# cvlab-kaist/CoPoNeRF

Measured on AMD Instinct MI355X. Metric: rendered rays/sec (RealEstate10K-shaped 256x256 stereo pair, full-image render, 64 samples/ray), higher is better.
Workload: dtype f16 (fp16-input/fp32-accumulate MFMA for the per-sample MLPs; f32 decoder; f64 geometry island); 1 GPU; configs[1]: 256x256 stereo pair (narrow rig), full-image render 65536 rays x 64 samples, 1 pair(s) per GPU, render path only (z/rel_pose/flow given, val=True); chunk_rays=65536, lanes=1, pairs_per_gpu=1

## Files before the change

### coponerf_amd/csrc/attend_units.hip

```cpp
#include <algorithm>

#include "hid_sum.h"
#include "local_units_body.h"

namespace {

constexpr int HC = 1664;
constexpr int NCHUNK = HC / 8;
constexpr int NL = 4;
constexpr int NS = 2 * TG;
constexpr int AU_THREADS = (NL + NS) * 64;
constexpr int RU = HID_BLOCK_ROWS;
constexpr int LDS_MAX = 160 * 1024;

__device__ __forceinline__ float wave_max(float v) {
#pragma unroll
    for (int o = 32; o > 0; o >>= 1) v = fmaxf(v, __shfl_xor(v, o));
    return v;
}
__device__ __forceinline__ float wave_sum(float v) {
#pragma unroll
    for (int o = 32; o > 0; o >>= 1) v += __shfl_xor(v, o);
    return v;
}
__device__ __forceinline__ void group_barrier() {
    asm volatile("s_waitcnt lgkmcnt(0)" ::: "memory");
    __builtin_amdgcn_s_barrier();
    asm volatile("" ::: "memory");
}

struct GroupUnits {
    unsigned lw, upg, upw, nmy, bid, nwg;
    __device__ __forceinline__ unsigned niter() const { return nmy * upw; }
    __device__ __forceinline__ unsigned unit(unsigned it, int, bool& live) const {
        it = min(it, nmy * upw - 1);
        const unsigned k = it / upw, idx = lw + (it - k * upw) * NL;
        live = idx < upg;
        return (bid + k * nwg) * upg + min(idx, upg - 1);
    }
    __device__ __forceinline__ void after(unsigned it) const {
        if ((it + 1) % upw == 0) group_barrier();
    }
};
struct RingLogits {
    float* ring;
    float* __restrict__ logits;
    unsigned lw, upw, nsblk;
    int S, T, a, fg;
    __device__ __forceinline__ void operator()(unsigned it, int, long long srow, float d) const {
        if (srow < 0 || fg != 0) return;
        const unsigned k = it / upw, idx = lw + (it - k * upw) * NL;
        const int v = (int)(idx / nsblk), s = (int)(idx % nsblk) * TSW + (a >> 2);
        ring[(k & 1) * (TG * T) + (a & 3) * T + v * S + s] = d;
        if (logits) logits[srow] = d;
    }
};

template <int MODE>
__global__ __launch_bounds__(AU_THREADS, 3) void attend_units_kernel(UnitArgs args, UnitGeo geo, const __half* __restrict__ hid,
                                                                     __half* __restrict__ hbar, float* __restrict__ at_wt,
                                                                     float* __restrict__ logits) {
    extern __shared__ __attribute__((aligned(16))) char smem[];
    constexpr size_t WB = 8 * 4 * 64 * sizeof(half8);
    UnitLds L;
    L.w2l = reinterpret_cast<half8*>(smem);
    L.wkl = reinterpret_cast<half8*>(smem + WB);
    L.b2s = reinterpret_cast<float*>(smem + 2 * WB);
    L.bks = L.b2s + 128;
    L.w1s = reinterpret_cast<half4*>(L.bks + 128);
    const int V = geo.V, R = geo.R, S = geo.S, T = V * S;
    float* ring = reinterpret_cast<float*>(smem + unit_lds_bytes<MODE>());
    float* wbuf = ring + 2 * TG * T;
    const int lane = threadIdx.x & 63;
    const int wave = __builtin_amdgcn_readfirstlane((int)(threadIdx.x >> 6));

    unit_stage_weights<MODE>(L, args, (int)threadIdx.x, AU_THREADS);
    __syncthreads();

    const unsigned upg = (unsigned)(V * geo.nsblk);
    const unsigned ngroups = (unsigned)geo.nunits / upg;
    const unsigned bid = blockIdx.x, nwg = gridDim.x;
    const unsigned nmy = (ngroups - bid + nwg - 1) / nwg;

    if (wave < NL) {
        const unsigned upw = (upg + NL - 1) / NL;
        GroupUnits seq{(unsigned)wave, upg, upw, nmy, bid, nwg};
        RingLogits sink{ring, logits, (unsigned)wave, upw, (unsigned)geo.nsblk, S, T, lane & 15, lane >> 4};
        unit_walk<MODE, 1>(L, args, geo, lane, seq, sink);
        return;
    }

    __builtin_amdgcn_s_setprio(1);
    const int sw = wave - NL, j = sw >> 1, half = sw & 1;
    constexpr int CPW = NCHUNK / 2;
    const int c0 = half * CPW + lane, c1 = half * CPW + min(64 + lane, CPW - 1);
    const bool live1 = lane < CPW - 64;
    const unsigned off0 = (unsigned)c0 * 8, off1 = (unsigned)c1 * 8;
    const int npair = T / (2 * RU);
    struct Ray {
        bool live;
        int b, r;
        size_t lray;
        const __half* hp;
    };
    auto ray_of = [&](unsigned k) {
        Ray o;
        const long long gq = geo.group0 + bid + (long long)k * nwg;
        o.b = (int)(gq / geo.groups_per_b);
        o.r = (int)(gq % geo.groups_per_b) * TG + j;
        const long long rayrel = (long long)o.b * R + o.r - geo.ray0;
        o.live = k < nmy && o.r < R && rayrel >= 0 && rayrel < geo.nrays;
        o.lray = (size_t)max(0LL, min(rayrel, (long long)geo.nrays - 1));
        o.hp = hid + o.lray * T * HC;
        return o;
    };
    auto issue = [&](const Ray& ray, half8 (&h0)[RU], half8 (&h1)[RU], int row) {
#pragma unroll
        for (int u = 0; u < RU; ++u) {
            const __half* rp = ray.hp + (size_t)(row + u) * HC;
            h0[u] = __builtin_nontemporal_load(reinterpret_cast<const half8*>(rp + off0));
            h1[u] = __builtin_nontemporal_load(reinterpret_cast<const half8*>(rp + off1));
        }
    };
    auto pin = [] {
        asm volatile("" ::: "memory");
        __builtin_amdgcn_sched_barrier(0);
    };
    half8 a0[RU], a1[RU], b0[RU], b1[RU];
    Ray nxt = ray_of(0);
    if (nxt.live && npair > 0) issue(nxt, a0, a1, 0);
    for (unsigned k = 0; k < nmy; ++k) {
        const Ray ray = nxt;
        nxt = ray_of(k + 1);
        const bool pre = nxt.live && npair > 0;
        const int b = ray.b, r = ray.r;
        group_barrier();
        if (!ray.live) {
            if (pre) issue(nxt, a0, a1, 0);
            continue;
        }

        const float* lg = ring + (k & 1) * (TG * T) + j * T;
        float* wt = wbuf + j * T;
        float lmax = -INFINITY;
        for (int row = lane; row < T; row += 64) lmax = fmaxf(lmax, lg[row] / 11.31f);
        const float gmax = wave_max(lmax);
        float ps[4] = {0.f, 0.f, 0.f, 0.f};
        for (int base = 0; base < T; base += 256) {
#pragma unroll
            for (int q = 0; q < 4; ++q) {
                const int row = base + q * 64 + lane;
                if (row < T) ps[q] += __expf(lg[row] / 11.31f - gmax);
            }
        }
#pragma unroll
        for (int q = 0; q < 4; ++q) ps[q] = wave_sum(ps[q]);
        const float inv = 1.0f / ((ps[0] + ps[1]) + (ps[2] + ps[3]));
        for (int row = lane; row < T; row += 64) {
            const float w = __expf(lg[row] / 11.31f - gmax) * inv;
            wt[row] = w;
            if (at_wt && half == 0) {
                const int v = row / S, s = row - v * S;
                at_wt[(((size_t)(b * V + v)) * R + r) * S + s] = w;
            }
        }
        asm volatile("s_waitcnt lgkmcnt(0)" ::: "memory");

        float acc0[8] = {0, 0, 0, 0, 0, 0, 0, 0}, acc1[8] = {0, 0, 0, 0, 0, 0, 0, 0};
        auto consume = [&](const half8 (&h0)[RU], const half8 (&h1)[RU], int row) {
#pragma unroll
            for (int u = 0; u < RU; ++u) {
                const float w = wt[row + u];
                hid_row_acc<true>(acc0, w, h0[u]);
                hid_row_acc<true>(acc1, w, h1[u]);
            }
        };
        if (npair > 0) {
            for (int p = 0; p + 1 < npair; ++p) {
                issue(ray, b0, b1, (2 * p + 1) * RU);
                pin();
                consume(a0, a1, 2 * p * RU);
                pin();
                issue(ray, a0, a1, (2 * p + 2) * RU);
                pin();
                consume(b0, b1, (2 * p + 1) * RU);
                pin();
            }
            issue(ray, b0, b1, (2 * npair - 1) * RU);
            pin();
            consume(a0, a1, (2 * npair - 2) * RU);
            pin();
            if (pre) issue(nxt, a0, a1, 0);
            pin();
            consume(b0, b1, (2 * npair - 1) * RU);
            pin();
        }
        for (int row = npair * 2 * RU; row < T; ++row) {
            const half8 h0 = __builtin_nontemporal_load(reinterpret_cast<const half8*>(ray.hp + (size_t)row * HC + off0));
            const half8 h1 = __builtin_nontemporal_load(reinterpret_cast<const half8*>(ray.hp + (size_t)row * HC + off1));
            const float w = wt[row];
            if (row < T - T % HID_BLOCK_ROWS) {
                hid_row_acc<true>(acc0, w, h0);
                hid_row_acc<true>(acc1, w, h1);
            } else {
                hid_row_acc<false>(acc0, w, h0);
                hid_row_acc<false>(acc1, w, h1);
            }
        }
        half8 o0, o1;
#pragma unroll
        for (int e = 0; e < 8; ++e) {
            o0[e] = (_Float16)acc0[e];
            o1[e] = (_Float16)acc1[e];
        }
        *reinterpret_cast<half8*>(hbar + ray.lray * HC + c0 * 8) = o0;
        if (live1) *reinterpret_cast<half8*>(hbar + ray.lray * HC + c1 * 8) = o1;
    }
}

template <int MODE>
int launch(const UnitArgs& args, const UnitGeo& geo, const __half* hid, __half* hbar, float* at_wt, float* logits, hipStream_t stream) {
    const int T = geo.V * geo.S;
    const size_t lds = unit_lds_bytes<MODE>() + (size_t)3 * TG * T * sizeof(float);
    CPN_REQUIRE(lds <= (size_t)LDS_MAX, CPN_E_SHAPE,
                "cpn_attend_units: V*S = %d needs %zu B of LDS (weights + 3 x 4 rays of logits / weights), the CU has %d", T, lds, LDS_MAX);
    auto kern = attend_units_kernel<MODE>;
    static bool attr_set = false;
    if (!attr_set) {
        hipError_t e = hipFuncSetAttribute((const void*)kern, hipFuncAttributeMaxDynamicSharedMemorySize, LDS_MAX);
        if (e != hipSuccess) {
            cpn_set_error("cpn_attend_units: cannot reserve %d B of LDS: %s", LDS_MAX, hipGetErrorString(e));
            return (int)e;
        }
        attr_set = true;
    }
    const long long ngroups = geo.nunits / (geo.V * geo.nsblk);
    const int num_cu = cpn_stream_cus((void*)stream);
    const unsigned grid = (unsigned)std::min<long long>(ngroups, num_cu);
    hipLaunchKernelGGL(kern, dim3(grid), dim3(AU_THREADS), lds, stream, args, geo, hid, hbar, at_wt, logits);
    CPN_LAUNCH_CHECK("cpn_attend_units");
    return 0;
}

}

extern "C" int cpn_attend_units(int mode, const float* loc8, const float* coords9, const float* w1, int ldw1, const float* b1,
                                const float* add, const uint16_t* w2, int ldw2, const float* b2, const uint16_t* wk2, int ldwk2,
                                const float* bk2, const float* w1b, int ldw1b, const float* b1b, const uint16_t* kh_u,
                                const uint16_t* hid, int B, int V, int R, int S, int ray0, int nrays, const float* lv_u,
                                uint16_t* hbar, float* at_wt, float* logits, void* stream) {
    CPN_REQUIRE(mode == 0 || mode == 2, CPN_E_ARG, "cpn_attend_units: mode must be 0 or 2 (got %d)", mode);
    CPN_REQUIRE(loc8 && coords9 && w1 && b1 && w2 && b2 && wk2 && bk2 && hid && hbar, CPN_E_ARG, "cpn_attend_units: null pointer");
    CPN_REQUIRE(mode == 0 ? kh_u != nullptr : (add && w1b && b1b), CPN_E_ARG, "cpn_attend_units: null pointer for mode %d", mode);
    CPN_REQUIRE(B > 0 && V == 2 && R > 0 && S > 0 && ldw1 >= 16 && ldw2 >= 128 && (ldw2 % 8) == 0 && ldwk2 >= 128 &&
                    (ldwk2 % 8) == 0 && (mode != 2 || ldw1b >= 16), CPN_E_SHAPE, "cpn_attend_units: bad shape");
    CPN_REQUIRE(ray0 >= 0 && nrays > 0 && (long long)ray0 + nrays <= (long long)B * R, CPN_E_ARG,
                "cpn_attend_units: ray range outside B*R");
    CPN_REQUIRE(((uintptr_t)kh_u % 16) == 0 && ((uintptr_t)w2 % 16) == 0 && ((uintptr_t)wk2 % 16) == 0 && ((uintptr_t)w1 % 16) == 0 &&
                    ((uintptr_t)w1b % 16) == 0 && ((uintptr_t)lv_u % 16) == 0 && ((uintptr_t)hid % 16) == 0 && ((uintptr_t)hbar % 16) == 0,
                CPN_E_ARG, "cpn_attend_units: fp16 operands, first-layer weights, hid and hbar must be 16-byte aligned");
    const UnitGeo geo = unit_geo(V, R, S, ray0, nrays);
    CPN_REQUIRE(geo.nunits * 16 < (1LL << 31), CPN_E_SHAPE, "cpn_attend_units: chunk too large for 32-bit indexing");
    const f32x4* lv_chunk = lv_u ? reinterpret_cast<const f32x4*>(lv_u) + (size_t)geo.group0 * V * geo.nsblk * 64 : nullptr;
    const UnitArgs args{loc8, coords9, w1, ldw1, b1, add, (const __half*)w2, ldw2, b2, (const __half*)wk2, ldwk2, bk2, w1b, ldw1b, b1b,
                        (const __half*)kh_u, nullptr, lv_chunk};
    return mode == 0 ? launch<0>(args, geo, (const __half*)hid, (__half*)hbar, at_wt, logits, (hipStream_t)stream)
                     : launch<2>(args, geo, (const __half*)hid, (__half*)hbar, at_wt, logits, (hipStream_t)stream);
}
```

### coponerf_amd/csrc/local_units_body.h

```cpp
#pragma once
#include "encode_common.h"

#ifndef CPN_LU_ABLATE
#define CPN_LU_ABLATE 0
#endif

namespace {

struct UnitGeo {
    int V, R, S, ray0, nrays, nsblk, groups_per_b;
    long long group0, nunits;
};

__host__ inline UnitGeo unit_geo(int V, int R, int S, int ray0, int nrays) {
    UnitGeo geo;
    geo.V = V; geo.R = R; geo.S = S; geo.ray0 = ray0; geo.nrays = nrays;
    geo.nsblk = (int)cpn_cdiv(S, TSW);
    geo.groups_per_b = (int)cpn_cdiv(R, TG);
    const int b_lo = ray0 / R, b_hi = (ray0 + nrays - 1) / R;
    geo.group0 = (long long)b_lo * geo.groups_per_b + (ray0 - b_lo * R) / TG;
    const long long group1 = (long long)b_hi * geo.groups_per_b + (ray0 + nrays - 1 - b_hi * R) / TG;
    geo.nunits = (group1 - geo.group0 + 1) * V * geo.nsblk;
    return geo;
}

struct UnitArgs {
    const float* loc8; const float* coords9;
    const float* w1; int ldw1; const float* b1; const float* add;
    const __half* w2; int ldw2; const float* b2;
    const __half* wk2; int ldwk2; const float* bk2;
    const float* w1b; int ldw1b; const float* b1b;
    const __half* kh_u; __half* ce_u; const f32x4* lv_u;
};

struct UnitLds {
    half8* w2l; half8* wkl; float* b2s; float* bks; half4* w1s;
};
template <int MODE>
__host__ __device__ constexpr size_t unit_lds_bytes() {
    return (size_t)(MODE != 1 ? 2 : 1) * 8 * 4 * 64 * sizeof(half8) + 2 * 128 * sizeof(float) + (size_t)(MODE == 2 ? 4 : 2) * 8 * 64 * sizeof(half4);
}

template <bool RELU>
__device__ __forceinline__ half8 pack_tiles(const f32x4& lo, const f32x4& hi) {
    half8 out;
#pragma unroll
    for (int q = 0; q < 4; ++q) {
        const f32x4& src = q < 2 ? lo : hi;
        const f32x2v two = {src[2 * (q & 1)], src[2 * (q & 1) + 1]};
        half2v hv = __builtin_convertvector(two, half2v);
        if (RELU) hv = __builtin_elementwise_max(hv, (half2v){(_Float16)0.0f, (_Float16)0.0f});
        out[2 * q] = hv[0];
        out[2 * q + 1] = hv[1];
    }
    return out;
}

template <int MODE>
__device__ __forceinline__ void unit_stage_weights(const UnitLds& L, const UnitArgs& A, int tid, int nthreads) {
    const int lane = tid & 63;
    const int a = lane & 15, fg = lane >> 4;
    for (int i = tid; i < 8 * 4 * 64; i += nthreads) {
        const int l = i & 63, p = (i >> 6) & 3, t = i >> 8;
        const int ch = (t >> 1) * 32 + ((l & 15) >> 2) * 8 + (t & 1) * 4 + (l & 3);
        L.w2l[i] = *reinterpret_cast<const half8*>(A.w2 + (size_t)ch * A.ldw2 + p * 32 + (l >> 4) * 8);
        if constexpr (MODE != 1) L.wkl[i] = *reinterpret_cast<const half8*>(A.wk2 + (size_t)ch * A.ldwk2 + p * 32 + (l >> 4) * 8);
    }
    if (tid < 128) {
        L.b2s[tid] = A.b2[tid];
        L.bks[tid] = MODE != 1 ? A.bk2[tid] : 0.0f;
    }
    if (tid < 64) {
        auto split = [&](const float* wsrc, int ldw, const float* bsrc, int ch, half4& hi, half4& lo) {
            f32x4 wv = *reinterpret_cast<const f32x4*>(wsrc + (size_t)ch * ldw + fg * 4);
            if (fg == 0) wv[3] = bsrc[ch];
#pragma unroll
            for (int i = 0; i < 4; ++i) {
                hi[i] = (_Float16)wv[i];
                lo[i] = (_Float16)(wv[i] - (float)hi[i]);
            }
        };
#pragma unroll
        for (int t = 0; t < 8; ++t) {
            const int ch = (t >> 1) * 32 + (a >> 2) * 8 + (t & 1) * 4 + (a & 3);
            half4 hi, lo;
            split(A.w1, A.ldw1, A.b1, ch, hi, lo);
            L.w1s[(0 * 8 + t) * 64 + lane] = hi;
            L.w1s[(1 * 8 + t) * 64 + lane] = lo;
            if constexpr (MODE == 2) {
                split(A.w1b, A.ldw1b, A.b1b, ch, hi, lo);
                L.w1s[(2 * 8 + t) * 64 + lane] = hi;
                L.w1s[(3 * 8 + t) * 64 + lane] = lo;
            }
        }
    }
}

template <int MODE, int U, class Seq, class Sink>
__device__ __forceinline__ void unit_walk(const UnitLds& L, const UnitArgs& A, const UnitGeo& geo, const int lane, Seq& seq,
                                          Sink& sink) {
    const int a = lane & 15, fg = lane >> 4;
    const int V = geo.V, R = geo.R, S = geo.S;
    const float* __restrict__ loc8 = A.loc8;
    const float* __restrict__ coords9 = A.coords9;
    const float* __restrict__ add = A.add;
    const __half* __restrict__ kh_u = A.kh_u;
    __half* __restrict__ ce_u = A.ce_u;
    const f32x4* __restrict__ lv_u = A.lv_u;

    struct RowIn {
        f32x4 lv;
        unsigned rayrel;
        long long srow;
    };
    auto fetch = [&](unsigned uu) {
        const int sblk = (int)(uu % (unsigned)geo.nsblk);
        const int v = (int)((uu / (unsigned)geo.nsblk) % (unsigned)V);
        const long long gq = geo.group0 + uu / ((unsigned)geo.nsblk * (unsigned)V);
        const int b = (int)(gq / geo.groups_per_b), rgroup = (int)(gq % geo.groups_per_b);
        const RowId id = tile_row(a, rgroup, sblk, S, R, b, geo.ray0, geo.nrays);
        const int r = min(id.r, R - 1), s = min(id.s, S - 1);
        const size_t nr = ((size_t)(b * V + v)) * R + r;
        const float* lp = loc8 + (nr * S + s) * 8;
        const float* c9 = coords9 + nr * 9;
        RowIn o;
        const long long rayrel = (long long)b * R + r - geo.ray0;
        o.rayrel = (unsigned)max(0LL, min(rayrel, (long long)geo.nrays - 1));
        o.srow = id.live ? (rayrel * V + v) * S + s : -1;
        if (lv_u) {
            o.lv = __builtin_nontemporal_load(lv_u + (size_t)uu * 64 + lane);
            return o;
        }
        if (fg == 0) { const f32x4 l0 = *reinterpret_cast<const f32x4*>(lp); o.lv = f32x4{l0[0], l0[1], l0[2], 1.0f}; }
        else if (fg == 1) o.lv = f32x4{0.f, 0.f, c9[0], c9[1]};
        else if (fg == 2) o.lv = f32x4{c9[2], lp[3], lp[4], lp[5]};
        else o.lv = f32x4{lp[6], c9[6], c9[7], c9[8]};
        return o;
    };

    auto layer128 = [&](const half8* wfr, const float* bias_s, const half8 (&b)[U][4], f32x4 (&o)[U][8]) {
        constexpr int NF = 32, FD = 4;
        if (CPN_LU_ABLATE & 16) {
#pragma unroll
            for (int u = 0; u < U; ++u)
#pragma unroll
                for (int t = 0; t < 8; ++t) o[u][t] = f32x4{b[u][t & 3][0], b[u][t & 3][1], b[u][t & 3][2], b[u][t & 3][3]};
            return;
        }
        half8 af[FD];
#pragma unroll
        for (int d = 0; d < FD; ++d) af[d] = wfr[(((d & 7) * 4) + (d >> 3)) * 64 + lane];
#pragma unroll
        for (int t = 0; t < 8; ++t) {
            const f32x4 bv = *reinterpret_cast<const f32x4*>(bias_s + (t >> 1) * 32 + fg * 8 + (t & 1) * 4);
#pragma unroll
            for (int u = 0; u < U; ++u) o[u][t] = bv;
        }
#pragma unroll
        for (int i = 0; i < NF; ++i) {
            const int t = i & 7, pblk = i >> 3;
#pragma unroll
            for (int u = 0; u < U; ++u) o[u][t] = __builtin_amdgcn_mfma_f32_16x16x32_f16(af[i % FD], b[u][pblk], o[u][t], 0, 0, 0);
            if (i + FD < NF) af[i % FD] = wfr[((((i + FD) & 7) * 4) + ((i + FD) >> 3)) * 64 + lane];
        }
        __builtin_amdgcn_sched_group_barrier(0x100, FD + 8, 0);
#pragma unroll
        for (int i = 0; i < NF - FD; ++i) {
            __builtin_amdgcn_sched_group_barrier(0x008, U, 0);
            __builtin_amdgcn_sched_group_barrier(0x100, 1, 0);
        }
        __builtin_amdgcn_sched_group_barrier(0x008, FD * U, 0);
    };
    auto layer16 = [&](int ws, const half4 (&xh)[U], const half4 (&xl)[U], f32x4 (&o)[U][8]) {
#pragma unroll
        for (int t = 0; t < 8; ++t) {
            const half4 wh = L.w1s[(ws * 8 + t) * 64 + lane], wl = L.w1s[((ws + 1) * 8 + t) * 64 + lane];
#pragma unroll
            for (int u = 0; u < U; ++u) {
                o[u][t] = __builtin_amdgcn_mfma_f32_16x16x16f16(wl, xh[u], o[u][t], 0, 0, 0);
                o[u][t] = __builtin_amdgcn_mfma_f32_16x16x16f16(wh, xl[u], o[u][t], 0, 0, 0);
                o[u][t] = __builtin_amdgcn_mfma_f32_16x16x16f16(wh, xh[u], o[u][t], 0, 0, 0);
            }
        }
    };
    auto add_rows = [&](unsigned rayrel, f32x4 (&dst)[8]) {
#pragma unroll
        for (int t = 0; t < 8; ++t)
            dst[t] = (CPN_LU_ABLATE & 2) ? f32x4{0.f, 0.f, 0.f, 0.f}
                                         : *reinterpret_cast<const f32x4*>(add + (size_t)rayrel * 128 + (t >> 1) * 32 + fg * 8 + (t & 1) * 4);
    };

    const unsigned niter = seq.niter();
    if (niter == 0) return;
    RowIn cur[U];
    constexpr bool ADD_AHEAD = MODE == 2 && U == 1;
    f32x4 addn[ADD_AHEAD ? U : 1][8];
#pragma unroll
    for (int u = 0; u < U; ++u) {
        bool l0;
        cur[u] = fetch(seq.unit(0u, u, l0));
        if constexpr (ADD_AHEAD) add_rows(cur[u].rayrel, addn[u]);
    }
    for (unsigned it = 0; it < niter; ++it) {
        RowIn nxt[U];
        unsigned un[U];
        bool ulive[U];
#pragma unroll
        for (int u = 0; u < U; ++u) {
            bool ln;
            un[u] = seq.unit(it, u, ulive[u]);
            nxt[u] = (CPN_LU_ABLATE & 4) ? cur[u] : fetch(seq.unit(it + 1, u, ln));
        }
        half8 cv[U][4];
        if constexpr (MODE != 2) {
#pragma unroll
            for (int u = 0; u < U; ++u)
#pragma unroll
                for (int p = 0; p < 4; ++p)
                    cv[u][p] = (CPN_LU_ABLATE & 1) ? half8{} : __builtin_nontemporal_load(
                        reinterpret_cast<const half8*>(MODE == 0 ? kh_u : ce_u) + ((size_t)un[u] * 4 + p) * 64 + lane);
        }
        f32x4 acc[U][8];
        half4 xh[U], xl[U];
#pragma unroll
        for (int u = 0; u < U; ++u) {
#pragma unroll
            for (int t = 0; t < 8; ++t) acc[u][t] = f32x4{0.f, 0.f, 0.f, 0.f};
            if constexpr (ADD_AHEAD) {
#pragma unroll
                for (int t = 0; t < 8; ++t) acc[u][t] = addn[u][t];
                add_rows(nxt[u].rayrel, addn[u]);
            } else if constexpr (MODE != 0) {
                add_rows(cur[u].rayrel, acc[u]);
            }
#pragma unroll
            for (int i = 0; i < 4; ++i) {
                xh[u][i] = (_Float16)cur[u].lv[i];
                xl[u][i] = (_Float16)(cur[u].lv[i] - (float)xh[u][i]);
            }
        }
        if constexpr (MODE == 2) {
            f32x4 ab[U][8];
#pragma unroll
            for (int u = 0; u < U; ++u)
#pragma unroll
                for (int t = 0; t < 8; ++t) ab[u][t] = f32x4{0.f, 0.f, 0.f, 0.f};
            layer16(2, xh, xl, ab);
            half8 hq[U][4];
#pragma unroll
            for (int u = 0; u < U; ++u)
#pragma unroll
                for (int p = 0; p < 4; ++p) hq[u][p] = pack_tiles<true>(ab[u][2 * p], ab[u][2 * p + 1]);
            f32x4 oq[U][8];
            layer128(L.wkl, L.bks, hq, oq);
#pragma unroll
            for (int u = 0; u < U; ++u)
#pragma unroll
                for (int p = 0; p < 4; ++p) cv[u][p] = pack_tiles<false>(oq[u][2 * p], oq[u][2 * p + 1]);
        }
        layer16(0, xh, xl, acc);
        half8 hb[U][4];
#pragma unroll
        for (int u = 0; u < U; ++u)
#pragma unroll
            for (int p = 0; p < 4; ++p) hb[u][p] = pack_tiles<true>(acc[u][2 * p], acc[u][2 * p + 1]);
        f32x4 o2[U][8];
        layer128(L.w2l, L.b2s, hb, o2);
        long long srow[U];
        float dsum[U];
#pragma unroll
        for (int u = 0; u < U; ++u) {
            srow[u] = ulive[u] ? cur[u].srow : -1;
            cur[u] = nxt[u];
            dsum[u] = 0.0f;
        }
        if constexpr (MODE == 0) {
            half8 ce[U][4];
#pragma unroll
            for (int u = 0; u < U; ++u)
#pragma unroll
                for (int p = 0; p < 4; ++p) {
                    ce[u][p] = pack_tiles<false>(o2[u][2 * p], o2[u][2 * p + 1]);
                    if (ce_u && ulive[u] && !(CPN_LU_ABLATE & 8))
                        reinterpret_cast<half8*>(ce_u)[((size_t)un[u] * 4 + p) * 64 + lane] = ce[u][p];
                }
            f32x4 k2[U][8];
            layer128(L.wkl, L.bks, cv, k2);
#pragma unroll
            for (int u = 0; u < U; ++u)
#pragma unroll
                for (int p = 0; p < 4; ++p) {
                    const half8 kp = pack_tiles<false>(k2[u][2 * p], k2[u][2 * p + 1]);
#pragma unroll
                    for (int e = 0; e < 8; ++e) dsum[u] += (float)kp[e] * (float)ce[u][p][e];
                }
        } else {
#pragma unroll
            for (int u = 0; u < U; ++u)
#pragma unroll
                for (int p = 0; p < 4; ++p) {
                    const half8 qp = pack_tiles<false>(o2[u][2 * p], o2[u][2 * p + 1]);
#pragma unroll
                    for (int i = 0; i < 4; ++i) {
                        dsum[u] += (float)qp[i] * (float)cv[u][p][i];
                        dsum[u] += (float)qp[4 + i] * (float)cv[u][p][4 + i];
                    }
                }
        }
#pragma unroll
        for (int u = 0; u < U; ++u) {
            float d = dsum[u];
            d += __shfl_xor(d, 16);
            d += __shfl_xor(d, 32);
            sink(it, u, srow[u], d);
        }
        seq.after(it);
    }
}

}
```

Baseline: 2.906 million rays/s.

## Prefetch next ray's hid rows and kh fragments one step ahead via buffer loads

The weighted hidden-sum waves now use raw buffer loads with a per-ray resource whose size is zero for dead rays, so out-of-range loads return zero without branching. The double-buffered pipeline always prefetches both buffers of the next ray at the tail of the current one, rather than only the first half. The mode-0 logit waves also load the next unit's kh fragments one iteration ahead. Ablation macros are added as well. The aim is to hide global-load latency across ray and unit boundaries, at the cost of more live registers, which may reduce occupancy.

```diff
diff --git a/coponerf_amd/csrc/attend_units.hip b/coponerf_amd/csrc/attend_units.hip
--- a/coponerf_amd/csrc/attend_units.hip
+++ b/coponerf_amd/csrc/attend_units.hip
@@ -1,4 +1,11 @@
 #include <algorithm>
+
+#ifndef CPN_AU_ABLATE
+#define CPN_AU_ABLATE 0
+#endif
+#if (CPN_AU_ABLATE & 1) && !defined(CPN_LU_ABLATE)
+#define CPN_LU_ABLATE 1
+#endif
 
 #include "hid_sum.h"
 #include "local_units_body.h"
@@ -24,6 +31,7 @@
     return v;
 }
 __device__ __forceinline__ void group_barrier() {
+    if (CPN_AU_ABLATE & 4) return;
     asm volatile("s_waitcnt lgkmcnt(0)" ::: "memory");
     __builtin_amdgcn_s_barrier();
     asm volatile("" ::: "memory");
@@ -86,7 +94,7 @@
         const unsigned upw = (upg + NL - 1) / NL;
         GroupUnits seq{(unsigned)wave, upg, upw, nmy, bid, nwg};
         RingLogits sink{ring, logits, (unsigned)wave, upw, (unsigned)geo.nsblk, S, T, lane & 15, lane >> 4};
-        unit_walk<MODE, 1>(L, args, geo, lane, seq, sink);
+        unit_walk<MODE, 1, MODE == 0>(L, args, geo, lane, seq, sink);
         return;
     }
 
@@ -95,13 +103,14 @@
     constexpr int CPW = NCHUNK / 2;
     const int c0 = half * CPW + lane, c1 = half * CPW + min(64 + lane, CPW - 1);
     const bool live1 = lane < CPW - 64;
-    const unsigned off0 = (unsigned)c0 * 8, off1 = (unsigned)c1 * 8;
+    const int off0 = c0 * 16, off1 = c1 * 16;
     const int npair = T / (2 * RU);
     struct Ray {
         bool live;
         int b, r;
         size_t lray;
         const __half* hp;
+        int bytes;
     };
     auto ray_of = [&](unsigned k) {
         Ray o;
@@ -112,59 +121,65 @@
         o.live = k < nmy && o.r < R && rayrel >= 0 && rayrel < geo.nrays;
         o.lray = (size_t)max(0LL, min(rayrel, (long long)geo.nrays - 1));
         o.hp = hid + o.lray * T * HC;
+        o.bytes = o.live ? T * HC * (int)sizeof(__half) : 0;
         return o;
     };
-    auto issue = [&](const Ray& ray, half8 (&h0)[RU], half8 (&h1)[RU], int row) {
-#pragma unroll
-        for (int u = 0; u < RU; ++u) {
-            const __half* rp = ray.hp + (size_t)(row + u) * HC;
-            h0[u] = __builtin_nontemporal_load(reinterpret_cast<const half8*>(rp + off0));
-            h1[u] = __builtin_nontemporal_load(reinterpret_cast<const half8*>(rp + off1));
-        }
+    constexpr int NT_LOAD = 2;
+    auto rows_of = [](const Ray& ray) { return __builtin_amdgcn_make_buffer_rsrc((void*)ray.hp, 0, ray.bytes, 0x00020000); };
+    auto row_load = [&](const __amdgpu_buffer_rsrc_t& rs, int row, int off) {
+        return __builtin_bit_cast(half8, __builtin_amdgcn_raw_buffer_load_b128(rs, off, row * (HC * (int)sizeof(__half)), NT_LOAD));
     };
     auto pin = [] {
         asm volatile("" ::: "memory");
         __builtin_amdgcn_sched_barrier(0);
     };
+    auto issue = [&](const Ray& ray, half8 (&h0)[RU], half8 (&h1)[RU], int row) {
+        const __amdgpu_buffer_rsrc_t rs = rows_of(ray);
+#pragma unroll
+        for (int u = 0; u < RU; ++u) {
+            h0[u] = row_load(rs, row + u, off0);
+            h1[u] = row_load(rs, row + u, off1);
+        }
+        pin();
+    };
     half8 a0[RU], a1[RU], b0[RU], b1[RU];
     Ray nxt = ray_of(0);
-    if (nxt.live && npair > 0) issue(nxt, a0, a1, 0);
+    issue(nxt, a0, a1, 0);
+    issue(nxt, b0, b1, RU);
     for (unsigned k = 0; k < nmy; ++k) {
         const Ray ray = nxt;
         nxt = ray_of(k + 1);
-        const bool pre = nxt.live && npair > 0;
         const int b = ray.b, r = ray.r;
         group_barrier();
-        if (!ray.live) {
-            if (pre) issue(nxt, a0, a1, 0);
-            continue;
-        }
 
         const float* lg = ring + (k & 1) * (TG * T) + j * T;
-        float* wt = wbuf + j * T;
-        float lmax = -INFINITY;
-        for (int row = lane; row < T; row += 64) lmax = fmaxf(lmax, lg[row] / 11.31f);
-        const float gmax = wave_max(lmax);
-        float ps[4] = {0.f, 0.f, 0.f, 0.f};
-        for (int base = 0; base < T; base += 256) {
-#pragma unroll
-            for (int q = 0; q < 4; ++q) {
-                const int row = base + q * 64 + lane;
-                if (row < T) ps[q] += __expf(lg[row] / 11.31f - gmax);
-            }
-        }
-#pragma unroll
-        for (int q = 0; q < 4; ++q) ps[q] = wave_sum(ps[q]);
-        const float inv = 1.0f / ((ps[0] + ps[1]) + (ps[2] + ps[3]));
-        for (int row = lane; row < T; row += 64) {
-            const float w = __expf(lg[row] / 11.31f - gmax) * inv;
-            wt[row] = w;
-            if (at_wt && half == 0) {
-                const int v = row / S, s = row - v * S;
-                at_wt[(((size_t)(b * V + v)) * R + r) * S + s] = w;
-            }
-        }
-        asm volatile("s_waitcnt lgkmcnt(0)" ::: "memory");
+        float* wtw = wbuf + j * T;
+        const float* wt = (CPN_AU_ABLATE & 2) ? lg : wtw;
+        if (!(CPN_AU_ABLATE & 2)) {
+            float lmax = -INFINITY;
+            for (int row = lane; row < T; row += 64) lmax = fmaxf(lmax, lg[row] / 11.31f);
+            const float gmax = wave_max(lmax);
+            float ps[4] = {0.f, 0.f, 0.f, 0.f};
+            for (int base = 0; base < T; base += 256) {
+#pragma unroll
+                for (int q = 0; q < 4; ++q) {
+                    const int row = base + q * 64 + lane;
+                    if (row < T) ps[q] += __expf(lg[row] / 11.31f - gmax);
+                }
+            }
+#pragma unroll
+            for (int q = 0; q < 4; ++q) ps[q] = wave_sum(ps[q]);
+            const float inv = 1.0f / ((ps[0] + ps[1]) + (ps[2] + ps[3]));
+            for (int row = lane; row < T; row += 64) {
+                const float w = __expf(lg[row] / 11.31f - gmax) * inv;
+                wtw[row] = w;
+                if (at_wt && half == 0 && ray.live) {
+                    const int v = row / S, s = row - v * S;
+                    at_wt[(((size_t)(b * V + v)) * R + r) * S + s] = w;
+                }
+            }
+            asm volatile("s_waitcnt lgkmcnt(0)" ::: "memory");
+        }
 
         float acc0[8] = {0, 0, 0, 0, 0, 0, 0, 0}, acc1[8] = {0, 0, 0, 0, 0, 0, 0, 0};
         auto consume = [&](const half8 (&h0)[RU], const half8 (&h1)[RU], int row) {
@@ -174,30 +189,18 @@
                 hid_row_acc<true>(acc0, w, h0[u]);
                 hid_row_acc<true>(acc1, w, h1[u]);
             }
+            pin();
         };
-        if (npair > 0) {
-            for (int p = 0; p + 1 < npair; ++p) {
-                issue(ray, b0, b1, (2 * p + 1) * RU);
-                pin();
-                consume(a0, a1, 2 * p * RU);
-                pin();
-                issue(ray, a0, a1, (2 * p + 2) * RU);
-                pin();
-                consume(b0, b1, (2 * p + 1) * RU);
-                pin();
-            }
-            issue(ray, b0, b1, (2 * npair - 1) * RU);
-            pin();
-            consume(a0, a1, (2 * npair - 2) * RU);
-            pin();
-            if (pre) issue(nxt, a0, a1, 0);
-            pin();
-            consume(b0, b1, (2 * npair - 1) * RU);
-            pin();
+        for (int p = 0; p < npair; ++p) {
+            const bool last = p + 1 == npair;
+            const Ray& src = last ? nxt : ray;
+            consume(a0, a1, 2 * p * RU);
+            issue(src, a0, a1, last ? 0 : (2 * p + 2) * RU);
+            consume(b0, b1, (2 * p + 1) * RU);
+            issue(src, b0, b1, last ? RU : (2 * p + 3) * RU);
         }
         for (int row = npair * 2 * RU; row < T; ++row) {
-            const half8 h0 = __builtin_nontemporal_load(reinterpret_cast<const half8*>(ray.hp + (size_t)row * HC + off0));
-            const half8 h1 = __builtin_nontemporal_load(reinterpret_cast<const half8*>(ray.hp + (size_t)row * HC + off1));
+            const half8 h0 = row_load(rows_of(ray), row, off0), h1 = row_load(rows_of(ray), row, off1);
             const float w = wt[row];
             if (row < T - T % HID_BLOCK_ROWS) {
                 hid_row_acc<true>(acc0, w, h0);
@@ -213,8 +216,8 @@
             o0[e] = (_Float16)acc0[e];
             o1[e] = (_Float16)acc1[e];
         }
-        *reinterpret_cast<half8*>(hbar + ray.lray * HC + c0 * 8) = o0;
-        if (live1) *reinterpret_cast<half8*>(hbar + ray.lray * HC + c1 * 8) = o1;
+        if (ray.live) *reinterpret_cast<half8*>(hbar + ray.lray * HC + c0 * 8) = o0;
+        if (ray.live && live1) *reinterpret_cast<half8*>(hbar + ray.lray * HC + c1 * 8) = o1;
     }
 }
 
diff --git a/coponerf_amd/csrc/local_units_body.h b/coponerf_amd/csrc/local_units_body.h
--- a/coponerf_amd/csrc/local_units_body.h
+++ b/coponerf_amd/csrc/local_units_body.h
@@ -96,7 +96,7 @@
     }
 }
 
-template <int MODE, int U, class Seq, class Sink>
+template <int MODE, int U, bool KH_AHEAD = false, class Seq, class Sink>
 __device__ __forceinline__ void unit_walk(const UnitLds& L, const UnitArgs& A, const UnitGeo& geo, const int lane, Seq& seq,
                                           Sink& sink) {
     const int a = lane & 15, fg = lane >> 4;
@@ -195,24 +195,41 @@
     RowIn cur[U];
     constexpr bool ADD_AHEAD = MODE == 2 && U == 1;
     f32x4 addn[ADD_AHEAD ? U : 1][8];
+    static_assert(!KH_AHEAD || (MODE == 0 && U == 1), "KH_AHEAD: mode 0, one unit per wave");
+    half8 cvn[KH_AHEAD ? U : 1][4];
+    auto kh_frags = [&](unsigned uu, half8 (&dst)[4]) {
+#pragma unroll
+        for (int p = 0; p < 4; ++p)
+            dst[p] = (CPN_LU_ABLATE & 1) ? half8{} : __builtin_nontemporal_load(reinterpret_cast<const half8*>(kh_u) + ((size_t)uu * 4 + p) * 64 + lane);
+    };
 #pragma unroll
     for (int u = 0; u < U; ++u) {
         bool l0;
-        cur[u] = fetch(seq.unit(0u, u, l0));
+        const unsigned u0 = seq.unit(0u, u, l0);
+        cur[u] = fetch(u0);
         if constexpr (ADD_AHEAD) add_rows(cur[u].rayrel, addn[u]);
+        if constexpr (KH_AHEAD) kh_frags(u0, cvn[u]);
     }
     for (unsigned it = 0; it < niter; ++it) {
         RowIn nxt[U];
-        unsigned un[U];
+        unsigned un[U], un1[U];
         bool ulive[U];
 #pragma unroll
         for (int u = 0; u < U; ++u) {
             bool ln;
             un[u] = seq.unit(it, u, ulive[u]);
-            nxt[u] = (CPN_LU_ABLATE & 4) ? cur[u] : fetch(seq.unit(it + 1, u, ln));
+            un1[u] = seq.unit(it + 1, u, ln);
+            nxt[u] = (CPN_LU_ABLATE & 4) ? cur[u] : fetch(un1[u]);
         }
         half8 cv[U][4];
-        if constexpr (MODE != 2) {
+        if constexpr (KH_AHEAD) {
+#pragma unroll
+            for (int u = 0; u < U; ++u) {
+#pragma unroll
+                for (int p = 0; p < 4; ++p) cv[u][p] = cvn[u][p];
+                kh_frags(un1[u], cvn[u]);
+            }
+        } else if constexpr (MODE != 2) {
 #pragma unroll
             for (int u = 0; u < U; ++u)
 #pragma unroll
```

Result: slower. 2.872 million rays/s (-1.2%).
